# laomao0/BIN

Hardware: AMD Instinct MI355X
Metric: interpolated frames/sec at 1280x720 (higher is better)
Workload: dtype f16x3 (fp16 hi+lo pairs = 22-bit significands, 3 MFMA products, f32 accumulate; fp32-class: 1e-6 vs the fp32 reference); 1 GPU; Adobe240 test_blur 1280x720 inference, batch=1 per GPU (6-frame window padded to 768x1344 by the test.py rule), window-sharded; precision=f16x3, streams=1, pipelined_steps=False, four_call_schedule=False, parity=max-abs <= 2e-5 (f16x3) vs the fp32 reference (tests/)

## Files before the change

### bin_amd/csrc/binhip_fused_x3.hip

```cpp
#include "binhip_fused.h"
#include <type_traits>

namespace {

struct TX {
    static constexpr int R = 2, NW = 4, TH = 8, PH = 10, PW = 34;
    static constexpr int PP = (PH * PW * 2 + 63) / 64;
    static constexpr int CWP = 9, LWP = 3;
    static constexpr int PATCH_BYTES = PP * 1024;
    static constexpr int WPL = (CWP + LWP) * 1024;
    static constexpr int WBUF_BYTES = 2 * WPL;
    static constexpr int W_OFF = 2 * PATCH_BYTES;
    static constexpr int LDS_BYTES = W_OFF + 2 * WBUF_BYTES;
    static constexpr int NCHUNK = 12;
    static constexpr int NPJ = (PP + NW - 1) / NW;
    static constexpr int TAILW_OFF = W_OFF;
    static_assert(2 * LDS_BYTES <= 160 * 1024, "two workgroups per CU");
};

__device__ __forceinline__ half8 ld8(const char* p) { return *reinterpret_cast<const half8*>(p); }

__device__ __forceinline__ void tx_issue_patch(const TailKArgs& a, char* smem, int c, int pl, int wave, const unsigned* voff,
                                               long long plane_elems, unsigned plane_bytes) {
    __amdgpu_buffer_rsrc_t rs = __builtin_amdgcn_make_buffer_rsrc(
        (void*)((pl ? a.x_lo : a.x_hi) + (long long)c * plane_elems), 0, plane_bytes, 0x00020000);
    char* lds = smem + pl * TX::PATCH_BYTES;
#pragma unroll
    for (int j = 0; j < TX::NPJ; ++j) {
        const int i = wave + TX::NW * j;
        if (i < TX::PP) __builtin_amdgcn_raw_ptr_buffer_load_lds(rs, (lds_void_t*)(lds + i * 1024), 16, voff[j], 0, 0, 0);
    }
}

__device__ __forceinline__ void tx_issue_weights(const TailKArgs& a, char* smem, int c, int buf, int wave, int lane) {
    __amdgpu_buffer_rsrc_t ch = __builtin_amdgcn_make_buffer_rsrc((void*)(a.wc_hi + (long long)c * (9 * 32 * 16)), 0, 9 * 1024, 0x00020000);
    __amdgpu_buffer_rsrc_t cl = __builtin_amdgcn_make_buffer_rsrc((void*)(a.wc_lo + (long long)c * (9 * 32 * 16)), 0, 9 * 1024, 0x00020000);
    __amdgpu_buffer_rsrc_t lh = __builtin_amdgcn_make_buffer_rsrc((void*)(a.wl_hi + (long long)c * (96 * 16)), 0, 3 * 1024, 0x00020000);
    __amdgpu_buffer_rsrc_t ll = __builtin_amdgcn_make_buffer_rsrc((void*)(a.wl_lo + (long long)c * (96 * 16)), 0, 3 * 1024, 0x00020000);
    char* lds = smem + TX::W_OFF + buf * TX::WBUF_BYTES;
    const unsigned v = (unsigned)(lane * 16);
#pragma unroll
    for (int j = 0; j < 6; ++j) {
        const int i = wave + TX::NW * j;
        const int pl = i >= 12 ? 1 : 0;
        const int k = i - 12 * pl;
        const bool lff = k >= TX::CWP;
        const int t = lff ? k - TX::CWP : k;
        __builtin_amdgcn_raw_ptr_buffer_load_lds(pl ? (lff ? ll : cl) : (lff ? lh : ch), (lds_void_t*)(lds + i * 1024), 16, v,
                                                 t * 1024, 0, 0);
    }
}

__device__ __forceinline__ void tx_issue_tailw(const TailKArgs& a, char* smem, int wave, int lane) {
    __amdgpu_buffer_rsrc_t lh = __builtin_amdgcn_make_buffer_rsrc((void*)(a.wl_hi + (long long)12 * (96 * 16)), 0, 6 * 1024, 0x00020000);
    __amdgpu_buffer_rsrc_t ll = __builtin_amdgcn_make_buffer_rsrc((void*)(a.wl_lo + (long long)12 * (96 * 16)), 0, 6 * 1024, 0x00020000);
    char* lds = smem + TX::TAILW_OFF;
#pragma unroll
    for (int j = 0; j < 3; ++j) {
        const int i = wave + TX::NW * j;
        const int pl = i >= 6 ? 1 : 0;
        __builtin_amdgcn_raw_ptr_buffer_load_lds(pl ? ll : lh, (lds_void_t*)(lds + i * 1024), 16, (unsigned)(lane * 16),
                                                 (i - 6 * pl) * 1024, 0, 0);
    }
}

template <int RES>
__device__ __forceinline__ void tx_add_residual_row(const half8& bc, floatx16 (&accl)[3][TX::R], int r) {
    constexpr int K = RES >> 1, HF = RES & 1;
    union H8 { half8 h; unsigned u[4]; };
    H8 v;
    v.h = bc;
#pragma unroll
    for (int k = 0; k < 2; ++k) {
        auto sw = __builtin_amdgcn_permlane32_swap(v.u[k], v.u[2 + k], false, false);
        v.u[k] = sw[0]; v.u[2 + k] = sw[1];
    }
#pragma unroll
    for (int ge = 0; ge < 2; ++ge)
#pragma unroll
        for (int j = 0; j < 4; ++j) accl[K][r][4 * (2 * HF + ge) + j] += (float)v.h[4 * ge + j];
}

template <bool HI, int RES>
__device__ __forceinline__ void tx_compute(const char* pb, const char* wb, int a_lane_off, int b_lane_off,
                                           floatx16 (&accc)[TX::R], floatx16 (&accl)[3][TX::R], half8 (&carry)[TX::R]) {
    constexpr int R = TX::R;
    constexpr int NSTEP = 12;
    half8 B[2][R + 2];
    half8 Ah[2], Al[2];
    auto load_b = [&](int dx, half8 (&dst)[R + 2]) {
#pragma unroll
// ... 25 lines not shown
        if constexpr (RES >= 0) {
            if (s == 0) {
#pragma unroll
                for (int r = 0; r < R; ++r) tx_add_residual_row<RES>(carry[r], accl, r);
                __builtin_amdgcn_sched_barrier(0);
            }
        }
        if (!lff) {
            const int set = dx & 1;
            if constexpr (HI) {
#pragma unroll
                for (int r = 0; r < R; ++r)
                    accc[r] = __builtin_amdgcn_mfma_f32_32x32x16_f16(Al[s & 1], B[set][r + k], accc[r], 0, 0, 0);
            }
#pragma unroll
            for (int r = 0; r < R; ++r)
                accc[r] = __builtin_amdgcn_mfma_f32_32x32x16_f16(Ah[s & 1], B[set][r + k], accc[r], 0, 0, 0);
        } else {
            if constexpr (HI) {
#pragma unroll
                for (int r = 0; r < R; ++r)
                    accl[k][r] = __builtin_amdgcn_mfma_f32_32x32x16_f16(Al[s & 1], B[1][r + 1], accl[k][r], 0, 0, 0);
            }
#pragma unroll
            for (int r = 0; r < R; ++r)
                accl[k][r] = __builtin_amdgcn_mfma_f32_32x32x16_f16(Ah[s & 1], B[1][r + 1], accl[k][r], 0, 0, 0);
        }
        __builtin_amdgcn_sched_barrier(0);
    }
#pragma unroll
    for (int r = 0; r < R; ++r) carry[r] = B[1][r + 1];
}

__global__ void __launch_bounds__(256) __attribute__((amdgpu_waves_per_eu(2, 2)))
rdb_tail_x3_kernel(const TailKArgs a, const float* __restrict__ bias_c, const float* __restrict__ bias_l) {
    extern __shared__ __attribute__((aligned(16))) char smem[];
    BH_TL_DECL;
    BH_TL_BEGIN();
    const int tid = threadIdx.x;
    const int lane = tid & 63;
    const int wave = __builtin_amdgcn_readfirstlane(tid >> 6);
    const int n = lane & 31, kg = lane >> 5;

    int bid = blockIdx.x;
    if (a.xcd_remap) bid = xcd_band(bid, gridDim.x);
    const int tx = bid % a.tiles_x;
    bid /= a.tiles_x;
    const int ty = bid % a.tiles_y;
    const int img = bid / a.tiles_y;
    const int tx0 = tx * 32, ty0 = ty * TX::TH;
    const int H = a.H, W = a.W;
    const long long plane_elems = (long long)a.N * H * W * 16;
    const unsigned plane_bytes = (unsigned)(plane_elems * 2);

    unsigned voff[TX::NPJ];
#pragma unroll
    for (int j = 0; j < TX::NPJ; ++j) {
        const int i = wave + TX::NW * j;
        const int q = i * 64 + lane;
        const int cg = q >= TX::PH * TX::PW ? 1 : 0;
        const int p = q - cg * (TX::PH * TX::PW);
        const int py = p / TX::PW, px = p - py * TX::PW;
        const int gy = ty0 + py - 1, gx = tx0 + px - 1;
        const bool ok = (p < TX::PH * TX::PW) && gy >= 0 && gy < H && gx >= 0 && gx < W;
        voff[j] = ok ? (unsigned)((((long long)img * H + gy) * W + gx) * 32 + cg * 16) : 0x80000000u;
    }

    floatx16 accc[TX::R];
    floatx16 accl[3][TX::R];
#pragma unroll
    for (int r = 0; r < TX::R; ++r)
#pragma unroll
        for (int e = 0; e < 16; ++e) {
            accc[r][e] = 0.f;
            accl[0][r][e] = 0.f; accl[1][r][e] = 0.f; accl[2][r][e] = 0.f;
        }
    const int a_lane_off = n * 32 + ((kg ^ ((n >> 3) & 1)) << 4);
    const int b_lane_off = (kg * (TX::PH * TX::PW) + wave * TX::R * TX::PW + n) * 16;

    __builtin_amdgcn_s_setprio(2);
    tx_issue_weights(a, smem, 0, 0, wave, lane);
    tx_issue_patch(a, smem, 0, 0, wave, voff, plane_elems, plane_bytes);
    half8 carry[TX::R];
    auto chunk = [&](const int c, auto res_hi, auto res_lo) __attribute__((always_inline)) {
        constexpr int RH = decltype(res_hi)::value, RL = decltype(res_lo)::value;
        const char* wb = smem + TX::W_OFF + (c & 1) * TX::WBUF_BYTES;
        wait_vmcnt<0>();
        __builtin_amdgcn_s_barrier();
        __builtin_amdgcn_sched_barrier(0);
#if BINHIP_TIMELINE
        if (c == 0) BH_TL_STAMP(1);
#endif
        tx_issue_patch(a, smem, c, 1, wave, voff, plane_elems, plane_bytes);
        if (c + 1 < TX::NCHUNK) tx_issue_weights(a, smem, c + 1, (c + 1) & 1, wave, lane);
        else tx_issue_tailw(a, smem, wave, lane);
        tx_compute<true, RH>(smem, wb, a_lane_off, b_lane_off, accc, accl, carry);
        wait_vmcnt<0>();
        __builtin_amdgcn_s_barrier();
        __builtin_amdgcn_sched_barrier(0);
        if (c + 1 < TX::NCHUNK) tx_issue_patch(a, smem, c + 1, 0, wave, voff, plane_elems, plane_bytes);
        tx_compute<false, RL>(smem + TX::PATCH_BYTES, wb, a_lane_off, b_lane_off, accc, accl, carry);
    };
    using std::integral_constant;
    chunk(0, integral_constant<int, -1>{}, integral_constant<int, 0>{});
    chunk(1, integral_constant<int, 0>{}, integral_constant<int, 1>{});
    chunk(2, integral_constant<int, 1>{}, integral_constant<int, 2>{});
    chunk(3, integral_constant<int, 2>{}, integral_constant<int, 3>{});
    chunk(4, integral_constant<int, 3>{}, integral_constant<int, 4>{});
    chunk(5, integral_constant<int, 4>{}, integral_constant<int, 5>{});
    chunk(6, integral_constant<int, 5>{}, integral_constant<int, -1>{});
    for (int c = 7; c < TX::NCHUNK; ++c) chunk(c, integral_constant<int, -1>{}, integral_constant<int, -1>{});
    wait_vmcnt<0>();
    __builtin_amdgcn_s_barrier();
    __builtin_amdgcn_sched_barrier(0);

    __builtin_amdgcn_s_setprio(0);
    const int gx = tx0 + n;
    union H4 { half4 h; unsigned u[2]; };
    union H8 { half8 h; unsigned u[4]; };
    unsigned sat = 0;
    half8 Bh[2][TX::R], Bl[2][TX::R];
#pragma unroll
    for (int r = 0; r < TX::R; ++r) {
        const int gy = ty0 + wave * TX::R + r;
        const bool ok = (gy < H) && (gx < W);
#pragma unroll
        for (int gp = 0; gp < 2; ++gp) {
            H4 hv[2], lv[2];
#pragma unroll
            for (int ge = 0; ge < 2; ++ge) {
                const int g = 2 * gp + ge;
                float b8[8];
#pragma unroll
                for (int j = 0; j < 8; ++j) b8[j] = bias_c[8 * g + j];
                const float v[4] = {accc[r][4 * g + 0] + (kg ? b8[4] : b8[0]), accc[r][4 * g + 1] + (kg ? b8[5] : b8[1]),
                                    accc[r][4 * g + 2] + (kg ? b8[6] : b8[2]), accc[r][4 * g + 3] + (kg ? b8[7] : b8[3])};
                split_pair(v[0], v[1], sat, hv[ge].u[0], lv[ge].u[0], true);
                split_pair(v[2], v[3], sat, hv[ge].u[1], lv[ge].u[1], true);
            }
#pragma unroll
            for (int k = 0; k < 2; ++k) {
                auto sw = __builtin_amdgcn_permlane32_swap(hv[0].u[k], hv[1].u[k], false, false);
                hv[0].u[k] = sw[0]; hv[1].u[k] = sw[1];
                auto sl = __builtin_amdgcn_permlane32_swap(lv[0].u[k], lv[1].u[k], false, false);
                lv[0].u[k] = sl[0]; lv[1].u[k] = sl[1];
            }
            H8 fh, fl;
            fh.u[0] = hv[0].u[0]; fh.u[1] = hv[0].u[1]; fh.u[2] = hv[1].u[0]; fh.u[3] = hv[1].u[1];
            fl.u[0] = lv[0].u[0]; fl.u[1] = lv[0].u[1]; fl.u[2] = lv[1].u[0]; fl.u[3] = lv[1].u[1];
            Bh[gp][r] = fh.h;
            Bl[gp][r] = fl.h;
            if (a.o3_hi && ok) {
                const long long o = (long long)gp * plane_elems + ((((long long)img * H + gy) * W + gx) << 4) + kg * 8;
                *reinterpret_cast<uint4*>(a.o3_hi + o) = make_uint4(fh.u[0], fh.u[1], fh.u[2], fh.u[3]);
                *reinterpret_cast<uint4*>(a.o3_lo + o) = make_uint4(fl.u[0], fl.u[1], fl.u[2], fl.u[3]);
            }
        }
    }

    const char* tailw = smem + TX::TAILW_OFF;
#pragma unroll
    for (int t = 0; t < 2; ++t) {
#pragma unroll
        for (int mt = 0; mt < 3; ++mt) {
            const int off = (t * 96 + mt * 32) * 32 + a_lane_off;
            const half8 Ah = ld8(tailw + off);
            const half8 Al = ld8(tailw + 6 * 1024 + off);
#pragma unroll
            for (int r = 0; r < TX::R; ++r) {
                accl[mt][r] = __builtin_amdgcn_mfma_f32_32x32x16_f16(Al, Bh[t][r], accl[mt][r], 0, 0, 0);
                accl[mt][r] = __builtin_amdgcn_mfma_f32_32x32x16_f16(Ah, Bh[t][r], accl[mt][r], 0, 0, 0);
                accl[mt][r] = __builtin_amdgcn_mfma_f32_32x32x16_f16(Ah, Bl[t][r], accl[mt][r], 0, 0, 0);
            }
        }
    }
    if (a.flags && __builtin_amdgcn_ballot_w64(sat != 0) != 0 && lane == 0) atomicOr(a.flags, BINHIP_FLAG_SATURATED);
    BH_TL_STAMP(2);

    ConvKArgs e;
    e.bias = a.bl; e.y_hi = a.y_hi; e.y_lo = a.y_lo;
    e.r_hi = e.r_lo = e.r2_hi = e.r2_lo = e.m_hi = nullptr;
    e.flags = a.flags;
    e.N = a.N; e.H = H; e.W = W;
    e.relu = 0; e.has_res = 0; e.cout = 96; e.wt = a.wt;
    e.och_limit = 6; e.res_chunks = 0; e.mask_from = 0; e.y_cpg = 0; e.y_cpg_inv = 0; e.y_group_stride = 0; e.y_unshuf = 0;
    conv_epilogue<3, TX::R, 3, BINHIP_EPI_PLANES, false>(e, bias_l, accl, img, ty0 + wave * TX::R, tx0, 0, true, n, kg, plane_elems);
    BH_TL_FINISH(a, blockIdx.x);
}

}

int bh_launch_tail_x3(const TailKArgs& a0, hipStream_t s) {
    static std::atomic<unsigned long long> lds_set{0};
    if (int rc = bh_set_max_lds(&rdb_tail_x3_kernel, TX::LDS_BYTES, lds_set)) return rc;
    TailKArgs a = a0;
    a.tiles_x = (a.W + 31) / 32;
    a.tiles_y = (a.H + TX::TH - 1) / TX::TH;
#if BINHIP_TIMELINE
    a.tl = bh_tl_reserve((unsigned)(a.tiles_x * a.tiles_y * a.N), &a.tl_base);
    a.tl_launch = (2u << 24) | (g_bh_tl_serial.fetch_add(1) & 0xFFFFFFu);
#endif
    rdb_tail_x3_kernel<<<dim3((unsigned)(a.tiles_x * a.tiles_y * a.N)), dim3(256), TX::LDS_BYTES, s>>>(a, a.bc, a.bl);
    BH_CHECK_LAUNCH();
    return 0;
}
```

### bin_amd/csrc/binhip_conv_common.h

```cpp
#pragma once
#include "binhip_internal.h"
#ifndef BINHIP_TIMELINE
#define BINHIP_TIMELINE 0
#endif

typedef _Float16 half8 __attribute__((ext_vector_type(8)));
typedef _Float16 half4 __attribute__((ext_vector_type(4)));
typedef float floatx16 __attribute__((ext_vector_type(16)));
typedef float floatx4 __attribute__((ext_vector_type(4)));
typedef __attribute__((address_space(3))) void lds_void_t;
typedef unsigned u32x4 __attribute__((ext_vector_type(4)));

int bh_launch_upnet_ring(const void* x_hi, const void* x_lo, const float* wvar, const float* bvar, float* out, const float* const* images,
                         int nimg, int N, int H, int W, int cin, hipStream_t s);
int bh_upnet_gsub(const float* g, int N, int H, int W, const float* scale, void* y_hi, void* y_lo, void* status, hipStream_t s);
int bh_upnet_ring_dgrad(const float* g, const float* wvar, const float* scale, void* gx_hi, void* gx_lo, void* status, int N, int H, int W,
                        int cin, hipStream_t s);
int bh_upnet_ring_wgrad(const float* g, const void* x_hi, const void* x_lo, float* dwvar, float* dbvar, int N, int H, int W, int cin,
                        int accumulate, hipStream_t s);
struct ConvKArgs {
    const _Float16* x_hi;
    const _Float16* x_lo;
    const _Float16* w_hi;
    const _Float16* w_lo;
// ... 96 lines not shown
__device__ __forceinline__ void wait_vmcnt() {
    asm volatile("s_waitcnt vmcnt(%0)" ::"n"(N) : "memory");
}

__device__ __forceinline__ void store16(_Float16* base, long long off_elems, uint4 v, int wt) {
    if (wt) {
        __amdgpu_buffer_rsrc_t rs = __builtin_amdgcn_make_buffer_rsrc((void*)base, 0, 0xFFFFFFFFu, 0x00020000);
        u32x4 d = {v.x, v.y, v.z, v.w};
        __builtin_amdgcn_raw_buffer_store_b128(d, rs, (int)(off_elems * 2), 0, 16);
    } else {
        *reinterpret_cast<uint4*>(base + off_elems) = v;
    }
}

__device__ __forceinline__ int xcd_band(int bid, int nwg) {
    const int q = nwg >> 3, r = nwg & 7, xcd = bid & 7, k = bid >> 3;
    return (xcd < r ? xcd * (q + 1) : r * (q + 1) + (xcd - r) * q) + k;
}

template <int MT, int R, int NT, int EPI, bool XTRA>
__device__ __forceinline__ void conv_epilogue(const ConvKArgs& a, const float* __restrict__ bias, floatx16 (&acc)[MT][R],
                                              int img, int row0, int tx0, int co0, bool first_col, int n, int kg,
                                              long long plane_elems) {
    const int H = a.H, W = a.W;
    const int gx = tx0 + n;
    auto bias4 = [&](int co_u, float (&bv)[4]) {
        float b8[8];
#pragma unroll
        for (int j = 0; j < 8; ++j) b8[j] = bias[co_u + j];
#pragma unroll
        for (int j = 0; j < 4; ++j) bv[j] = kg ? b8[4 + j] : b8[j];
    };
    if constexpr (EPI == BINHIP_EPI_FINAL_SUBPIX) {
        const int ncolour = a.cout >> 2;
        const int H2 = 2 * H, W2 = 2 * W;
        float bv[2][4];
        bias4(co0, bv[0]);
        bias4(co0 + 8, bv[1]);
        const bool col_ok = first_col && (gx < W);
        float sum[R][2][4];
#pragma unroll
        for (int r = 0; r < R; ++r) {
            const int gy = row0 + r;
#pragma unroll
            for (int g = 0; g < 2; ++g) {
                const int c = 2 * g + kg;
                const bool ok = col_ok && gy < H && c < ncolour;
#pragma unroll
                for (int q = 0; q < 4; ++q) {
                    float sj = 0.f;
                    if (ok && a.nimg > 0) {
                        const long long idx = (((long long)img * ncolour + c) * H2 + 2 * gy + (q >> 1)) * W2 + 2 * gx + (q & 1);
                        sj = a.img[0][idx];
                        for (int t = 1; t < a.nimg; ++t) sj += a.img[t][idx];
                        sj = sj / (float)a.nimg;
                    }
                    sum[r][g][q] = sj;
                }
            }
        }
#pragma unroll
        for (int r = 0; r < R; ++r) {
            const int gy = row0 + r;
#pragma unroll
            for (int g = 0; g < 2; ++g) {
                const int c = 2 * g + kg;
                if (!(col_ok && gy < H && c < ncolour)) continue;
#pragma unroll
                for (int q = 0; q < 4; ++q) {
                    const long long idx = (((long long)img * ncolour + c) * H2 + 2 * gy + (q >> 1)) * W2 + 2 * gx + (q & 1);
                    a.out_f32[idx] = (acc[0][r][4 * g + q] + bv[g][q]) + sum[r][g][q];
                }
            }
        }
    } else if constexpr (EPI == BINHIP_EPI_FINAL) {
        float bv[4];
        bias4(co0, bv);
        const bool mine = (kg == 0) && first_col && (gx < W);
        float sum[R][4];
#pragma unroll
        for (int r = 0; r < R; ++r) {
            const int gy = row0 + r;
#pragma unroll
            for (int j = 0; j < 4; ++j) {
                float sj = 0.f;
                if (mine && gy < H && j < a.cout && a.nimg > 0) {
                    const long long idx = (((long long)img * a.cout + j) * H + gy) * W + gx;
                    sj = a.img[0][idx];
                    for (int t = 1; t < a.nimg; ++t) sj += a.img[t][idx];
                    sj = sj / (float)a.nimg;
                }
                sum[r][j] = sj;
            }
        }
#pragma unroll
        for (int r = 0; r < R; ++r) {
            const int gy = row0 + r;
            if (!(mine && gy < H)) continue;
#pragma unroll
            for (int j = 0; j < 4; ++j) {
                if (j >= a.cout) break;
                const long long idx = (((long long)img * a.cout + j) * H + gy) * W + gx;
                a.out_f32[idx] = (acc[0][r][j] + bv[j]) + sum[r][j];
            }
// ... 246 lines not shown
```

### bin_amd/csrc/binhip_conv_x3.hip

```cpp
#include "binhip_conv_common.h"
constexpr int X3_R = 2, X3_WN = 8;

template <int KS, int R, int WN>
struct X3Cfg {
    static constexpr int PAD = KS / 2;
    static constexpr int TH = R * WN;
    static constexpr int PH = TH + KS - 1;
    static constexpr int PW = 32 + KS - 1;
    static constexpr int PP = (PH * PW * 2 + 63) / 64;
    static constexpr int WP = KS * KS;
    static constexpr int NW = WN;
    static constexpr int PATCH_BYTES = PP * 1024;
    static constexpr int WBUF_BYTES = 2 * WP * 1024;
    static constexpr int LDS_BYTES = 2 * PATCH_BYTES + 2 * WBUF_BYTES;
    static constexpr int NPJ = (PP + NW - 1) / NW;
    static constexpr int NWJ = (2 * WP + NW - 1) / NW;
    static_assert((KS == 3 ? 2 : 1) * LDS_BYTES <= 160 * 1024, "LDS budget");
};

template <class C>
__device__ __forceinline__ void x3_issue_patch(const ConvKArgs& a, char* smem, int c, int pl, int buf, int wave,
                                               const unsigned* voff, long long plane_elems, unsigned plane_bytes) {
    const _Float16* xb = pl ? a.x_lo : a.x_hi;
    const long long coff = (a.cpg > 0) ? (long long)(c / a.cpg) * a.group_stride + (long long)(c % a.cpg) * plane_elems
                                       : (long long)c * plane_elems;
    __amdgpu_buffer_rsrc_t rs = __builtin_amdgcn_make_buffer_rsrc((void*)(xb + coff), 0, plane_bytes, 0x00020000);
    char* lds = smem + buf * C::PATCH_BYTES;
#pragma unroll
    for (int j = 0; j < C::NPJ; ++j) {
        const int i = wave + C::NW * j;
        if ((C::PP % C::NW == 0) || (i < C::PP))
            __builtin_amdgcn_raw_ptr_buffer_load_lds(rs, (lds_void_t*)(lds + i * 1024), 16, voff[j], 0, 0, 0);
    }
}

template <class C, int KS>
__device__ __forceinline__ void x3_issue_weights(const ConvKArgs& a, char* smem, int c, int buf, int wave, int lane, int z) {
    const long long woff = ((long long)z * a.nchunks + c) * (KS * KS * 32 * 16);
    __amdgpu_buffer_rsrc_t wh = __builtin_amdgcn_make_buffer_rsrc((void*)(a.w_hi + woff), 0, KS * KS * 1024, 0x00020000);
    __amdgpu_buffer_rsrc_t wl = __builtin_amdgcn_make_buffer_rsrc((void*)(a.w_lo + woff), 0, KS * KS * 1024, 0x00020000);
    char* lds = smem + 2 * C::PATCH_BYTES + buf * C::WBUF_BYTES;
#pragma unroll
    for (int j = 0; j < C::NWJ; ++j) {
        const int i = wave + C::NW * j;
        if (((2 * C::WP) % C::NW == 0) || (i < 2 * C::WP)) {
            const bool lo = i >= C::WP;
            const int t = lo ? i - C::WP : i;
            __builtin_amdgcn_raw_ptr_buffer_load_lds(lo ? wl : wh, (lds_void_t*)(lds + i * 1024), 16,
                                                     (unsigned)(lane * 16), t * 1024, 0, 0);
        }
    }
}

__device__ __forceinline__ half8 x3_ld8(const char* p) { return *reinterpret_cast<const half8*>(p); }
__device__ __forceinline__ floatx16 x3_mfma(half8 a, half8 b, floatx16 c) {
    return __builtin_amdgcn_mfma_f32_32x32x16_f16(a, b, c, 0, 0, 0);
}

template <class C, int KS, int R, bool HI>
__device__ __forceinline__ void x3_compute(const char* pb, const char* wb, int a_lane_off, int b_lane_off, floatx16 (&acc)[R]) {
    constexpr int NTAP = KS * KS;
    half8 B[2][R + KS - 1];
    half8 Ah[2], Al[2];
    auto load_b = [&](int dx, half8 (&dst)[R + KS - 1]) {
#pragma unroll
        for (int rr = 0; rr < R + KS - 1; ++rr) dst[rr] = x3_ld8(pb + b_lane_off + (rr * C::PW + dx) * 16);
    };
    auto load_a = [&](int s, half8& h, half8& l) {
        const int dx = s / KS, dy = s % KS;
        const int off = ((dy * KS + dx) * 32) * 32 + a_lane_off;
        h = x3_ld8(wb + off);
        if constexpr (HI) l = x3_ld8(wb + C::WP * 1024 + off);
    };
    load_b(0, B[0]);
    load_a(0, Ah[0], Al[0]);
#pragma unroll
    for (int s = 0; s < NTAP; ++s) {
        const int dx = s / KS, dy = s % KS;
        if (s + 1 < NTAP) load_a(s + 1, Ah[(s + 1) & 1], Al[(s + 1) & 1]);
        if (dy == 0 && dx + 1 < KS) load_b(dx + 1, B[(dx + 1) & 1]);
        __builtin_amdgcn_sched_barrier(0);
        if constexpr (HI) {
#pragma unroll
// ... 69 lines not shown
    const int n = lane & 31;
    const int kg = lane >> 5;
    const int tx0 = tx * 32, ty0 = ty * C::TH;
    const int H = a.H, W = a.W;
    const long long plane_elems = (long long)a.N * H * W * 16;
    const unsigned plane_bytes = (unsigned)(plane_elems * 2);

    unsigned voff[C::NPJ];
#pragma unroll
    for (int j = 0; j < C::NPJ; ++j) {
        const int i = wave + C::NW * j;
        const int q = i * 64 + lane;
        const int cg = q >= C::PH * C::PW ? 1 : 0;
        const int p = q - cg * (C::PH * C::PW);
        const int py = p / C::PW;
        const int px = p - py * C::PW;
        const int gy = ty0 + py - C::PAD;
        const int gx = tx0 + px - C::PAD;
        const bool ok = (p < C::PH * C::PW) && (gy >= 0) && (gy < H) && (gx >= 0) && (gx < W);
        voff[j] = ok ? (unsigned)((((long long)img * H + gy) * W + gx) * 32 + cg * 16) : 0x80000000u;
    }

    floatx16 acc[1][R];
#pragma unroll
    for (int r = 0; r < R; ++r)
#pragma unroll
        for (int e = 0; e < 16; ++e) acc[0][r][e] = 0.f;

    const int nchunks = a.nchunks;
    const int a_lane_off = n * 32 + ((kg ^ ((n >> 3) & 1)) << 4);
    const int b_lane_off = (kg * (C::PH * C::PW) + wave * R * C::PW + n) * 16;

    __builtin_amdgcn_s_setprio(2);
    x3_issue_weights<C, KS>(a, smem, 0, 0, wave, lane, z);
    if constexpr (GATED) {
        if (gate.chunk <= 0 && gate.flags) {
            if (tid < 9) {
                const int ny = ty + tid / 3 - 1, nx = tx + tid % 3 - 1;
                if (ny >= 0 && ny < a.tiles_y && nx >= 0 && nx < a.tiles_x) {
                    const unsigned* f = gate.flags + ((size_t)img * a.tiles_y + ny) * a.tiles_x + nx;
                    unsigned spins = 0;
                    while (__hip_atomic_load(f, __ATOMIC_RELAXED, __HIP_MEMORY_SCOPE_AGENT) != gate.epoch) {
                        __builtin_amdgcn_s_sleep(2);
                        if (++spins > RDB3_SPIN_LIMIT) {
                            if (gate.status) atomicOr(gate.status, BINHIP_STATUS_SYNC_TIMEOUT);
                            break;
                        }
                    }
                }
            }
            __builtin_amdgcn_s_barrier();
            __builtin_amdgcn_sched_barrier(0);
        }
    }
    x3_issue_patch<C>(a, smem, 0, 0, 0, wave, voff, plane_elems, plane_bytes);
    for (int c = 0; c < nchunks; ++c) {
        const char* wb = smem + 2 * C::PATCH_BYTES + (c & 1) * C::WBUF_BYTES;
        if (a.prog_prio) {
            const int q = (4 * c) / nchunks;
            if (q == 0) __builtin_amdgcn_s_setprio(3);
            else if (q == 1) __builtin_amdgcn_s_setprio(2);
            else if (q == 2) __builtin_amdgcn_s_setprio(1);
            else __builtin_amdgcn_s_setprio(0);
        }
        wait_vmcnt<0>();
        __builtin_amdgcn_s_barrier();
        __builtin_amdgcn_sched_barrier(0);
#if BINHIP_TIMELINE
        if (c == 0) BH_TL_STAMP(1);
#endif
        x3_issue_patch<C>(a, smem, c, 1, 1, wave, voff, plane_elems, plane_bytes);
        if (c + 1 < nchunks) x3_issue_weights<C, KS>(a, smem, c + 1, (c + 1) & 1, wave, lane, z);
        unsigned gate_seen = gate.epoch;
        const unsigned* gate_word = nullptr;
        if constexpr (GATED) {
            if (c + 1 == gate.chunk && gate.flags && tid < 9) {
                const int ny = ty + tid / 3 - 1, nx = tx + tid % 3 - 1;
                if (ny >= 0 && ny < a.tiles_y && nx >= 0 && nx < a.tiles_x) {
                    gate_word = gate.flags + ((size_t)img * a.tiles_y + ny) * a.tiles_x + nx;
                    gate_seen = __hip_atomic_load(gate_word, __ATOMIC_RELAXED, __HIP_MEMORY_SCOPE_AGENT);
                }
            }
        }
        const bool pair = (KS == 5) && !XTRA && a.half_last && (c + 1 == nchunks);
        if constexpr (KS == 5 && !XTRA) {
            if (pair) x3_compute_pair<C, KS, R, true>(smem, wb, n, kg, wave, acc[0]);
            else x3_compute<C, KS, R, true>(smem, wb, a_lane_off, b_lane_off, acc[0]);
        } else {
            x3_compute<C, KS, R, true>(smem, wb, a_lane_off, b_lane_off, acc[0]);
        }
        wait_vmcnt<0>();
        __builtin_amdgcn_s_barrier();
        __builtin_amdgcn_sched_barrier(0);
        if constexpr (GATED) {
            if (c + 1 == gate.chunk && gate.flags) {
                if (gate_word) {
                    unsigned spins = 0;
                    while (gate_seen != gate.epoch) {
                        __builtin_amdgcn_s_sleep(2);
                        gate_seen = __hip_atomic_load(gate_word, __ATOMIC_RELAXED, __HIP_MEMORY_SCOPE_AGENT);
                        if (++spins > RDB3_SPIN_LIMIT) {
                            if (gate.status) atomicOr(gate.status, BINHIP_STATUS_SYNC_TIMEOUT);
                            break;
                        }
                    }
                }
                __builtin_amdgcn_s_barrier();
                __builtin_amdgcn_sched_barrier(0);
            }
        }
        if (c + 1 < nchunks) x3_issue_patch<C>(a, smem, c + 1, 0, 0, wave, voff, plane_elems, plane_bytes);
        if constexpr (KS == 5 && !XTRA) {
            if (pair) x3_compute_pair<C, KS, R, false>(smem + C::PATCH_BYTES, wb, n, kg, wave, acc[0]);
            else x3_compute<C, KS, R, false>(smem + C::PATCH_BYTES, wb, a_lane_off, b_lane_off, acc[0]);
        } else {
            x3_compute<C, KS, R, false>(smem + C::PATCH_BYTES, wb, a_lane_off, b_lane_off, acc[0]);
        }
    }
    BH_TL_STAMP(2);
    __builtin_amdgcn_s_setprio(0);
    conv_epilogue<1, R, 3, EPI, XTRA>(a, bias, acc, img, ty0 + wave * R, tx0, z * 32, z == 0, n, kg, plane_elems);
    BH_TL_FINISH(a, (((img * a.tiles_y + ty) * a.tiles_x + tx) * a.ncol + z));
}

template <int KS, int R, int WN, int EPI, int WIDE, bool XTRA>
__global__ void __launch_bounds__(64 * WN)
    __attribute__((amdgpu_waves_per_eu((KS == 5 && !XTRA) ? WN / 4 : WN / 2, (KS == 5 && !XTRA) ? WN / 4 : WN / 2)))
conv_x3_kernel(const ConvKArgs a, const float* __restrict__ bias) {
    extern __shared__ __attribute__((aligned(16))) char smem[];
    int bid = blockIdx.x;
    if (a.xcd_remap) bid = xcd_band(bid, gridDim.x);
    const int ncol = a.ncol;
    const int z = bid % ncol;
    bid /= ncol;
    const int tx = bid % a.tiles_x;
    bid /= a.tiles_x;
    const int ty = bid % a.tiles_y;
    const int img = bid / a.tiles_y;
    x3_tile<KS, R, WN, EPI, XTRA>(a, bias, smem, img, ty, tx, z);
}

struct Rdb3Args {
    ConvKArgs conv[3];
    unsigned* flags;
    unsigned epoch;
    int T;
};

template <int R, int WN>
__global__ void __launch_bounds__(64 * WN) __attribute__((amdgpu_waves_per_eu(WN / 2, WN / 2)))
conv_x3_rdbs_kernel(const Rdb3Args a, const float* __restrict__ bias0, const float* __restrict__ bias1,
                    const float* __restrict__ bias2) {
    extern __shared__ __attribute__((aligned(16))) char smem[];
    const int tiles_x = a.conv[0].tiles_x, tiles_y = a.conv[0].tiles_y;
    const int G = (int)gridDim.x;
    const int b = xcd_band((int)blockIdx.x, G);
#pragma unroll 1
    for (int p = 0; p < 3; ++p) {
        const ConvKArgs& ka = a.conv[p];
        const float* bias = p == 0 ? bias0 : (p == 1 ? bias1 : bias2);
        X3Gate gate;
        gate.flags = p > 0 ? a.flags + (size_t)(p - 1) * a.T : nullptr;
        gate.epoch = a.epoch;
        gate.chunk = ka.nchunks - 2;
        gate.status = ka.flags;
#pragma unroll 1
        for (int t0 = b; t0 < a.T; t0 += G) {
            int t = t0;
            const int tx = t % tiles_x;
            t /= tiles_x;
            const int ty = t % tiles_y;
            const int img = t / tiles_y;
            x3_tile<3, R, WN, BINHIP_EPI_PLANES, false, true>(ka, bias, smem, img, ty, tx, 0, gate);
            asm volatile("s_waitcnt vmcnt(0)" ::: "memory");
            __syncthreads();
            if (threadIdx.x == 0 && p < 2)
                __hip_atomic_store(a.flags + (size_t)p * a.T + t0, a.epoch, __ATOMIC_RELAXED, __HIP_MEMORY_SCOPE_AGENT);
        }
    }
}

template <int KS, int R, int WN, int EPI, int WIDE, bool XTRA>
static int launch_x3_x(const ConvKArgs& ka, int cout_pad, hipStream_t s) {
    using C = X3Cfg<KS, R, WN>;
    static std::atomic<unsigned long long> lds_set{0};
    if (int rc = bh_set_max_lds(&conv_x3_kernel<KS, R, WN, EPI, WIDE, XTRA>, C::LDS_BYTES, lds_set)) return rc;
    ConvKArgs a = ka;
    a.tiles_x = (a.W + 31) / 32;
    a.tiles_y = (a.H + C::TH - 1) / C::TH;
    a.ncol = cout_pad / 32;
    dim3 grid((unsigned)(a.tiles_x * a.tiles_y * a.N * a.ncol));
    a.prog_prio = (KS == 3 && !XTRA && (long long)grid.x <= 2ll * binhip_device_cus()) ? 1 : 0;
#if BINHIP_TIMELINE
    a.tl = bh_tl_reserve(grid.x, &a.tl_base);
    a.tl_launch = ((KS == 3 && EPI == BINHIP_EPI_PLANES && WIDE == 0 && !XTRA ? 1u : 3u) << 24) | (g_bh_tl_serial.fetch_add(1) & 0xFFFFFFu);
#endif
    conv_x3_kernel<KS, R, WN, EPI, WIDE, XTRA><<<grid, dim3(64 * C::NW), C::LDS_BYTES, s>>>(a, a.bias);
    BH_CHECK_LAUNCH();
    return 0;
}
template <int KS, int R, int WN, int EPI, int WIDE>
static int launch_x3(const ConvKArgs& ka, int cout_pad, hipStream_t s) {
    if constexpr (EPI == BINHIP_EPI_PLANES) {
        if (ka.has_res || ka.r2_hi || ka.m_hi || ka.y_unshuf) return launch_x3_x<KS, R, WN, EPI, WIDE, true>(ka, cout_pad, s);
    }
    return launch_x3_x<KS, R, WN, EPI, WIDE, false>(ka, cout_pad, s);
}

int bh_launch_rdb3_x3(const ConvKArgs* convs, unsigned* flags, unsigned epoch, int cus, hipStream_t s) {
    using C = X3Cfg<3, X3_R, X3_WN>;
    static std::atomic<unsigned long long> lds_set{0};
    static std::atomic<int> per_cu{-1};
    if (int rc = bh_set_max_lds(&conv_x3_rdbs_kernel<X3_R, X3_WN>, C::LDS_BYTES, lds_set)) return rc;
    int occ = per_cu.load(std::memory_order_acquire);
    if (occ < 0) {
        int n = 0;
        hipError_t e = hipOccupancyMaxActiveBlocksPerMultiprocessor(&n, conv_x3_rdbs_kernel<X3_R, X3_WN>, 64 * C::NW,
                                                                    C::LDS_BYTES);
        if (e != hipSuccess) return (int)e;
        occ = n > 2 ? 2 : n;
        per_cu.store(occ, std::memory_order_release);
    }
// ... 305 lines not shown

int bh_launch_final_m16(const ConvKArgs& ka, hipStream_t s) {
    using C = X3Cfg<3, 2, 8>;
    static std::atomic<unsigned long long> lds_set{0};
    if (ka.nchunks * 9 > M16::WPIECES * 8) return BINHIP_E_SHAPE;
    if (int rc = bh_set_max_lds(&final_m16_kernel, M16::LDS_BYTES, lds_set)) return rc;
    ConvKArgs a = ka;
    a.tiles_x = (a.W + 31) / 32;
    a.tiles_y = (a.H + C::TH - 1) / C::TH;
    a.ncol = 1;
    final_m16_kernel<<<dim3((unsigned)(a.tiles_x * a.tiles_y * a.N)), dim3(512), M16::LDS_BYTES, s>>>(a, a.bias);
    BH_CHECK_LAUNCH();
    return 0;
}

int bh_launch_final_dot2(const ConvKArgs& ka, hipStream_t s) {
    using C = X3Cfg<3, 2, 4>;
    ConvKArgs a = ka;
    a.tiles_x = (a.W + 31) / 32;
    a.tiles_y = (a.H + C::TH - 1) / C::TH;
    a.ncol = 1;
    dim3 grid((unsigned)(a.tiles_x * a.tiles_y * a.N));
    const unsigned* wh = reinterpret_cast<const unsigned*>(a.w_hi);
    final_dot2_kernel<1><<<grid, dim3(256), 2 * C::PATCH_BYTES, s>>>(a, wh, wh);
    BH_CHECK_LAUNCH();
    return 0;
}

int bh_launch_conv_x3_k5(const ConvKArgs& a, int cout_pad, hipStream_t s) {
    return launch_x3<5, X3_R, X3_WN, BINHIP_EPI_PLANES, 1>(a, cout_pad, s);
}

int bh_launch_conv_x3_k5_subpix(const ConvKArgs& a, hipStream_t s) {
    return launch_x3<5, X3_R, X3_WN, BINHIP_EPI_FINAL_SUBPIX, 0>(a, 32, s);
}

struct RingArgs {
    const _Float16* x_hi;
    const _Float16* x_lo;
    const float* wvar;
    const float* bvar;
    float* out;
    const float* img[5];
    int N, H, W, cin, nimg;
};
constexpr int RING_THREADS = 128;
__global__ void __launch_bounds__(RING_THREADS) upnet_ring_kernel(const RingArgs a) {
    __shared__ float red[3][RING_THREADS / 64];
    const int tid = threadIdx.x, lane = tid & 63, wave = tid >> 6;
    const int H = a.H, W = a.W, H2 = 2 * H, W2 = 2 * W;
    const int ring = 2 * W2 + 2 * (H2 - 2);
    int id = blockIdx.x;
    const int img = id / ring;
    id -= img * ring;
    int Y, X;
    if (id < W2) { Y = 0; X = id; }
    else if (id < 2 * W2) { Y = H2 - 1; X = id - W2; }
    else { const int k = id - 2 * W2; Y = 1 + (k >> 1); X = (k & 1) ? W2 - 1 : 0; }
    const int y = Y >> 1, i = Y & 1, x = X >> 1, j = X & 1;
    const int vy = (Y == 0) ? 0 : (Y == H2 - 1 ? 2 : 1), vx = (X == 0) ? 0 : (X == W2 - 1 ? 2 : 1);
    const int var = 3 * vy + vx, sub = 2 * i + j;
    const int cin = a.cin, ng = cin >> 3, items = 25 * ng;
    const long long wstride = (long long)25 * cin;
    const float* w = a.wvar + ((long long)var * 12 + sub) * wstride;
    float s0 = 0.f, s1 = 0.f, s2 = 0.f;
    for (int it = tid; it < items; it += RING_THREADS) {
        const int tap = it / ng, ci = (it - tap * ng) << 3;
// ... 65 lines not shown
```

Measured before the change: 16.27 interpolated frames/s.

## Deepen tail kernel patch ring to three slots for two-ahead prefetch

Turns the RDB tail x3 kernel's patch double buffer into a templated ring of two or three slots. The three-slot version packs each slot to the exact plane size and trims the last load piece to fit. It prefetches two sub-stages ahead and waits on partial vmcnt counts instead of draining all loads, so global latency overlaps the MFMA work. The host checks occupancy and falls back to the two-slot kernel if three slots would drop below two workgroups per CU; the cost is more LDS and fragile per-wave vmcnt bookkeeping.

```diff
diff --git a/bin_amd/csrc/binhip_fused_x3.hip b/bin_amd/csrc/binhip_fused_x3.hip
--- a/bin_amd/csrc/binhip_fused_x3.hip
+++ b/bin_amd/csrc/binhip_fused_x3.hip
@@ -7,40 +7,57 @@
     static constexpr int R = 2, NW = 4, TH = 8, PH = 10, PW = 34;
     static constexpr int PP = (PH * PW * 2 + 63) / 64;
     static constexpr int CWP = 9, LWP = 3;
-    static constexpr int PATCH_BYTES = PP * 1024;
+    static constexpr int PLANE_BYTES = PH * PW * 32;
+    static constexpr int LAST_LANES = (PLANE_BYTES - (PP - 1) * 1024) / 16;
     static constexpr int WPL = (CWP + LWP) * 1024;
     static constexpr int WBUF_BYTES = 2 * WPL;
-    static constexpr int W_OFF = 2 * PATCH_BYTES;
-    static constexpr int LDS_BYTES = W_OFF + 2 * WBUF_BYTES;
     static constexpr int NCHUNK = 12;
     static constexpr int NPJ = (PP + NW - 1) / NW;
+    static constexpr int WJ = 6, TWJ = 3;
+    static_assert(NW * (NPJ - 1) <= PP - 1 && PP - 1 < NW * NPJ, "only a wave's last patch piece can be the short one");
+    static_assert(WJ * NW == 2 * (CWP + LWP) && TWJ * NW == 4 * LWP, "weight pieces divide evenly over the waves");
+};
+
+template <int NSLOT>
+struct TXL {
+    static_assert(NSLOT == 2 || NSLOT == 3, "patch ring of two (one sub-stage ahead) or three (two ahead) slots");
+    static constexpr bool PACKED = NSLOT == 3;
+    static constexpr int PATCH_BYTES = PACKED ? TX::PLANE_BYTES : TX::PP * 1024;
+    static constexpr int W_OFF = NSLOT * PATCH_BYTES;
+    static constexpr int LDS_BYTES = W_OFF + 2 * TX::WBUF_BYTES;
     static constexpr int TAILW_OFF = W_OFF;
+    static_assert(PATCH_BYTES % 16 == 0, "ds_read_b128 alignment of every slot");
     static_assert(2 * LDS_BYTES <= 160 * 1024, "two workgroups per CU");
 };
 
 __device__ __forceinline__ half8 ld8(const char* p) { return *reinterpret_cast<const half8*>(p); }
 
-__device__ __forceinline__ void tx_issue_patch(const TailKArgs& a, char* smem, int c, int pl, int wave, const unsigned* voff,
+template <bool PACKED>
+__device__ __forceinline__ void tx_issue_patch(const TailKArgs& a, char* lds, int c, int pl, int wave, int lane, const unsigned* voff,
                                                long long plane_elems, unsigned plane_bytes) {
     __amdgpu_buffer_rsrc_t rs = __builtin_amdgcn_make_buffer_rsrc(
         (void*)((pl ? a.x_lo : a.x_hi) + (long long)c * plane_elems), 0, plane_bytes, 0x00020000);
-    char* lds = smem + pl * TX::PATCH_BYTES;
 #pragma unroll
     for (int j = 0; j < TX::NPJ; ++j) {
         const int i = wave + TX::NW * j;
-        if (i < TX::PP) __builtin_amdgcn_raw_ptr_buffer_load_lds(rs, (lds_void_t*)(lds + i * 1024), 16, voff[j], 0, 0, 0);
-    }
-}
-
-__device__ __forceinline__ void tx_issue_weights(const TailKArgs& a, char* smem, int c, int buf, int wave, int lane) {
+        if (j < TX::NPJ - 1 || i < TX::PP - 1 || (!PACKED && i == TX::PP - 1)) {
+            __builtin_amdgcn_raw_ptr_buffer_load_lds(rs, (lds_void_t*)(lds + i * 1024), 16, voff[j], 0, 0, 0);
+        } else if (i == TX::PP - 1) {
+            if (lane < TX::LAST_LANES)
+                __builtin_amdgcn_raw_ptr_buffer_load_lds(rs, (lds_void_t*)(lds + i * 1024), 16, voff[j], 0, 0, 0);
+        }
+    }
+}
+
+__device__ __forceinline__ void tx_issue_weights(const TailKArgs& a, char* wring, int c, int buf, int wave, int lane) {
     __amdgpu_buffer_rsrc_t ch = __builtin_amdgcn_make_buffer_rsrc((void*)(a.wc_hi + (long long)c * (9 * 32 * 16)), 0, 9 * 1024, 0x00020000);
     __amdgpu_buffer_rsrc_t cl = __builtin_amdgcn_make_buffer_rsrc((void*)(a.wc_lo + (long long)c * (9 * 32 * 16)), 0, 9 * 1024, 0x00020000);
     __amdgpu_buffer_rsrc_t lh = __builtin_amdgcn_make_buffer_rsrc((void*)(a.wl_hi + (long long)c * (96 * 16)), 0, 3 * 1024, 0x00020000);
     __amdgpu_buffer_rsrc_t ll = __builtin_amdgcn_make_buffer_rsrc((void*)(a.wl_lo + (long long)c * (96 * 16)), 0, 3 * 1024, 0x00020000);
-    char* lds = smem + TX::W_OFF + buf * TX::WBUF_BYTES;
+    char* lds = wring + buf * TX::WBUF_BYTES;
     const unsigned v = (unsigned)(lane * 16);
 #pragma unroll
-    for (int j = 0; j < 6; ++j) {
+    for (int j = 0; j < TX::WJ; ++j) {
         const int i = wave + TX::NW * j;
         const int pl = i >= 12 ? 1 : 0;
         const int k = i - 12 * pl;
@@ -51,12 +68,11 @@
     }
 }
 
-__device__ __forceinline__ void tx_issue_tailw(const TailKArgs& a, char* smem, int wave, int lane) {
+__device__ __forceinline__ void tx_issue_tailw(const TailKArgs& a, char* lds, int wave, int lane) {
     __amdgpu_buffer_rsrc_t lh = __builtin_amdgcn_make_buffer_rsrc((void*)(a.wl_hi + (long long)12 * (96 * 16)), 0, 6 * 1024, 0x00020000);
     __amdgpu_buffer_rsrc_t ll = __builtin_amdgcn_make_buffer_rsrc((void*)(a.wl_lo + (long long)12 * (96 * 16)), 0, 6 * 1024, 0x00020000);
-    char* lds = smem + TX::TAILW_OFF;
-#pragma unroll
-    for (int j = 0; j < 3; ++j) {
+#pragma unroll
+    for (int j = 0; j < TX::TWJ; ++j) {
         const int i = wave + TX::NW * j;
         const int pl = i >= 6 ? 1 : 0;
         __builtin_amdgcn_raw_ptr_buffer_load_lds(pl ? ll : lh, (lds_void_t*)(lds + i * 1024), 16, (unsigned)(lane * 16),
@@ -148,8 +164,10 @@
     for (int r = 0; r < R; ++r) carry[r] = B[1][r + 1];
 }
 
+template <int NSLOT>
 __global__ void __launch_bounds__(256) __attribute__((amdgpu_waves_per_eu(2, 2)))
 rdb_tail_x3_kernel(const TailKArgs a, const float* __restrict__ bias_c, const float* __restrict__ bias_l) {
+    using L = TXL<NSLOT>;
     extern __shared__ __attribute__((aligned(16))) char smem[];
     BH_TL_DECL;
     BH_TL_BEGIN();
@@ -195,27 +213,50 @@
     const int b_lane_off = (kg * (TX::PH * TX::PW) + wave * TX::R * TX::PW + n) * 16;
 
     __builtin_amdgcn_s_setprio(2);
-    tx_issue_weights(a, smem, 0, 0, wave, lane);
-    tx_issue_patch(a, smem, 0, 0, wave, voff, plane_elems, plane_bytes);
+    char* const wring = smem + L::W_OFF;
+    int slot = 0;
+    auto slot_base = [&](int k) { return smem + k * L::PATCH_BYTES; };
+    auto issue_plane = [&](int s, int k) __attribute__((always_inline)) {
+        tx_issue_patch<L::PACKED>(a, slot_base(k), s >> 1, s & 1, wave, lane, voff, plane_elems, plane_bytes);
+    };
+    const bool three = wave < TX::PP - 2 * TX::NW;
+    tx_issue_weights(a, wring, 0, 0, wave, lane);
+#pragma unroll
+    for (int s = 0; s < NSLOT - 1; ++s) issue_plane(s, s);
     half8 carry[TX::R];
     auto chunk = [&](const int c, auto res_hi, auto res_lo) __attribute__((always_inline)) {
         constexpr int RH = decltype(res_hi)::value, RL = decltype(res_lo)::value;
-        const char* wb = smem + TX::W_OFF + (c & 1) * TX::WBUF_BYTES;
-        wait_vmcnt<0>();
+        const char* wb = wring + (c & 1) * TX::WBUF_BYTES;
+        const bool last = c + 1 == TX::NCHUNK;
+        if constexpr (NSLOT == 3) {
+            if (three) wait_vmcnt<3>(); else wait_vmcnt<2>();
+        } else {
+            wait_vmcnt<0>();
+        }
         __builtin_amdgcn_s_barrier();
         __builtin_amdgcn_sched_barrier(0);
 #if BINHIP_TIMELINE
         if (c == 0) BH_TL_STAMP(1);
 #endif
-        tx_issue_patch(a, smem, c, 1, wave, voff, plane_elems, plane_bytes);
-        if (c + 1 < TX::NCHUNK) tx_issue_weights(a, smem, c + 1, (c + 1) & 1, wave, lane);
-        else tx_issue_tailw(a, smem, wave, lane);
-        tx_compute<true, RH>(smem, wb, a_lane_off, b_lane_off, accc, accl, carry);
-        wait_vmcnt<0>();
+        int prev = slot == 0 ? NSLOT - 1 : slot - 1;
+        if (NSLOT == 2 || !last) issue_plane(2 * c + NSLOT - 1, prev);
+        if (!last) tx_issue_weights(a, wring, c + 1, (c + 1) & 1, wave, lane);
+        else tx_issue_tailw(a, smem + L::TAILW_OFF, wave, lane);
+        tx_compute<true, RH>(slot_base(slot), wb, a_lane_off, b_lane_off, accc, accl, carry);
+        prev = slot;
+        slot = slot + 1 == NSLOT ? 0 : slot + 1;
+        if constexpr (NSLOT == 3) {
+            if (last) wait_vmcnt<3>();
+            else if (three) wait_vmcnt<9>();
+            else wait_vmcnt<8>();
+        } else {
+            wait_vmcnt<0>();
+        }
         __builtin_amdgcn_s_barrier();
         __builtin_amdgcn_sched_barrier(0);
-        if (c + 1 < TX::NCHUNK) tx_issue_patch(a, smem, c + 1, 0, wave, voff, plane_elems, plane_bytes);
-        tx_compute<false, RL>(smem + TX::PATCH_BYTES, wb, a_lane_off, b_lane_off, accc, accl, carry);
+        if (!last) issue_plane(2 * c + NSLOT, prev);
+        tx_compute<false, RL>(slot_base(slot), wb, a_lane_off, b_lane_off, accc, accl, carry);
+        slot = slot + 1 == NSLOT ? 0 : slot + 1;
     };
     using std::integral_constant;
     chunk(0, integral_constant<int, -1>{}, integral_constant<int, 0>{});
@@ -274,7 +315,7 @@
         }
     }
 
-    const char* tailw = smem + TX::TAILW_OFF;
+    const char* tailw = smem + L::TAILW_OFF;
 #pragma unroll
     for (int t = 0; t < 2; ++t) {
 #pragma unroll
@@ -306,9 +347,29 @@
 
 }
 
+template <int NSLOT>
+static int launch_tail_x3(TailKArgs& a, hipStream_t s) {
+    using L = TXL<NSLOT>;
+    rdb_tail_x3_kernel<NSLOT><<<dim3((unsigned)(a.tiles_x * a.tiles_y * a.N)), dim3(256), L::LDS_BYTES, s>>>(a, a.bc, a.bl);
+    BH_CHECK_LAUNCH();
+    return 0;
+}
+
 int bh_launch_tail_x3(const TailKArgs& a0, hipStream_t s) {
-    static std::atomic<unsigned long long> lds_set{0};
-    if (int rc = bh_set_max_lds(&rdb_tail_x3_kernel, TX::LDS_BYTES, lds_set)) return rc;
+    static std::atomic<unsigned long long> lds_set3{0}, lds_set2{0};
+    static std::atomic<int> per_cu{-1};
+    if (int rc = bh_set_max_lds(&rdb_tail_x3_kernel<3>, TXL<3>::LDS_BYTES, lds_set3)) return rc;
+    int occ = per_cu.load(std::memory_order_acquire);
+    if (occ < 0) {
+        int n = 0;
+        hipError_t e = hipOccupancyMaxActiveBlocksPerMultiprocessor(&n, rdb_tail_x3_kernel<3>, 256, TXL<3>::LDS_BYTES);
+        if (e != hipSuccess) return (int)e;
+        occ = n;
+        per_cu.store(occ, std::memory_order_release);
+    }
+    if (occ < 2) {
+        if (int rc = bh_set_max_lds(&rdb_tail_x3_kernel<2>, TXL<2>::LDS_BYTES, lds_set2)) return rc;
+    }
     TailKArgs a = a0;
     a.tiles_x = (a.W + 31) / 32;
     a.tiles_y = (a.H + TX::TH - 1) / TX::TH;
@@ -316,7 +377,5 @@
     a.tl = bh_tl_reserve((unsigned)(a.tiles_x * a.tiles_y * a.N), &a.tl_base);
     a.tl_launch = (2u << 24) | (g_bh_tl_serial.fetch_add(1) & 0xFFFFFFu);
 #endif
-    rdb_tail_x3_kernel<<<dim3((unsigned)(a.tiles_x * a.tiles_y * a.N)), dim3(256), TX::LDS_BYTES, s>>>(a, a.bc, a.bl);
-    BH_CHECK_LAUNCH();
-    return 0;
-}
+    return occ >= 2 ? launch_tail_x3<3>(a, s) : launch_tail_x3<2>(a, s);
+}
```

Result: no change. 16.22 interpolated frames/s (-0.3%).

## Compute sub-pixel final conv as a 4x4 window per output quad instead of 5x5

Applied to the files above, without the earlier changes.

The final 5x5 conv followed by pixel shuffle is recomputed with a 4x4 tap window, shifting the output quad by one pixel. Each lane gathers a phase-specific subset of the 5x5 weights, so 16 taps are processed instead of 25, cutting MFMA work and weight/patch traffic. The one-pixel border ring is left unwritten here, presumably filled by the existing upnet ring kernel. Pairs of outputs are stored as swapped float2 writes.

```diff
diff --git a/bin_amd/csrc/binhip_conv_common.h b/bin_amd/csrc/binhip_conv_common.h
--- a/bin_amd/csrc/binhip_conv_common.h
+++ b/bin_amd/csrc/binhip_conv_common.h
@@ -152,12 +152,18 @@
         for (int j = 0; j < 4; ++j) bv[j] = kg ? b8[4 + j] : b8[j];
     };
     if constexpr (EPI == BINHIP_EPI_FINAL_SUBPIX) {
+        constexpr int SH = (NT == 3) ? 1 : 0;
         const int ncolour = a.cout >> 2;
         const int H2 = 2 * H, W2 = 2 * W;
+        auto pix = [&](int c, int gy, int q) {
+            const int Y = SH ? 2 * gy + 2 - (q >> 1) : 2 * gy + (q >> 1);
+            const int X = SH ? 2 * gx + 2 - (q & 1) : 2 * gx + (q & 1);
+            return (((long long)img * ncolour + c) * H2 + Y) * W2 + X;
+        };
         float bv[2][4];
         bias4(co0, bv[0]);
         bias4(co0 + 8, bv[1]);
-        const bool col_ok = first_col && (gx < W);
+        const bool col_ok = first_col && (gx < W - SH);
         float sum[R][2][4];
 #pragma unroll
         for (int r = 0; r < R; ++r) {
@@ -165,12 +171,12 @@
 #pragma unroll
             for (int g = 0; g < 2; ++g) {
                 const int c = 2 * g + kg;
-                const bool ok = col_ok && gy < H && c < ncolour;
+                const bool ok = col_ok && gy < H - SH && c < ncolour;
 #pragma unroll
                 for (int q = 0; q < 4; ++q) {
                     float sj = 0.f;
                     if (ok && a.nimg > 0) {
-                        const long long idx = (((long long)img * ncolour + c) * H2 + 2 * gy + (q >> 1)) * W2 + 2 * gx + (q & 1);
+                        const long long idx = pix(c, gy, q);
                         sj = a.img[0][idx];
                         for (int t = 1; t < a.nimg; ++t) sj += a.img[t][idx];
                         sj = sj / (float)a.nimg;
@@ -185,11 +191,20 @@
 #pragma unroll
             for (int g = 0; g < 2; ++g) {
                 const int c = 2 * g + kg;
-                if (!(col_ok && gy < H && c < ncolour)) continue;
-#pragma unroll
-                for (int q = 0; q < 4; ++q) {
-                    const long long idx = (((long long)img * ncolour + c) * H2 + 2 * gy + (q >> 1)) * W2 + 2 * gx + (q & 1);
-                    a.out_f32[idx] = (acc[0][r][4 * g + q] + bv[g][q]) + sum[r][g][q];
+                if (!(col_ok && gy < H - SH && c < ncolour)) continue;
+                float v[4];
+#pragma unroll
+                for (int q = 0; q < 4; ++q) v[q] = (acc[0][r][4 * g + q] + bv[g][q]) + sum[r][g][q];
+                if constexpr (SH) {
+                    typedef float float2u __attribute__((ext_vector_type(2), aligned(4)));
+#pragma unroll
+                    for (int i = 0; i < 2; ++i) {
+                        float2u w = {v[2 * i + 1], v[2 * i]};
+                        *reinterpret_cast<float2u*>(a.out_f32 + pix(c, gy, 2 * i + 1)) = w;
+                    }
+                } else {
+#pragma unroll
+                    for (int q = 0; q < 4; ++q) a.out_f32[pix(c, gy, q)] = v[q];
                 }
             }
         }
diff --git a/bin_amd/csrc/binhip_conv_x3.hip b/bin_amd/csrc/binhip_conv_x3.hip
--- a/bin_amd/csrc/binhip_conv_x3.hip
+++ b/bin_amd/csrc/binhip_conv_x3.hip
@@ -3,7 +3,7 @@
 
 template <int KS, int R, int WN>
 struct X3Cfg {
-    static constexpr int PAD = KS / 2;
+    static constexpr int PAD = (KS == 4) ? 1 : KS / 2;
     static constexpr int TH = R * WN;
     static constexpr int PH = TH + KS - 1;
     static constexpr int PW = 32 + KS - 1;
@@ -16,6 +16,7 @@
     static constexpr int NPJ = (PP + NW - 1) / NW;
     static constexpr int NWJ = (2 * WP + NW - 1) / NW;
     static_assert((KS == 3 ? 2 : 1) * LDS_BYTES <= 160 * 1024, "LDS budget");
+    static_assert(KS != 4 || (PP == 21 && LDS_BYTES == 106 * 1024), "the 4 x 4 window of a 16 x 32 tile");
 };
 
 template <class C>
@@ -49,6 +50,26 @@
             __builtin_amdgcn_raw_ptr_buffer_load_lds(lo ? wl : wh, (lds_void_t*)(lds + i * 1024), 16,
                                                      (unsigned)(lane * 16), t * 1024, 0, 0);
         }
+    }
+}
+
+template <class C>
+__device__ __forceinline__ void x3_issue_weights_subpix(const ConvKArgs& a, char* smem, int c, int buf, int wave, int lane, int z) {
+    static_assert(C::WP == 16 && (2 * C::WP) % C::NW == 0, "4 x 4 taps, hi and lo");
+    const long long woff = ((long long)z * a.nchunks + c) * (25 * 32 * 16);
+    __amdgpu_buffer_rsrc_t wh = __builtin_amdgcn_make_buffer_rsrc((void*)(a.w_hi + woff), 0, 25 * 1024, 0x00020000);
+    __amdgpu_buffer_rsrc_t wl = __builtin_amdgcn_make_buffer_rsrc((void*)(a.w_lo + woff), 0, 25 * 1024, 0x00020000);
+    char* lds = smem + 2 * C::PATCH_BYTES + buf * C::WBUF_BYTES;
+    const int co = lane >> 1;
+    const int sub = co < 12 ? 5 * ((co >> 1) & 1) + (co & 1) : 0;
+    const unsigned voff = (unsigned)(lane * 16 + sub * 1024);
+#pragma unroll
+    for (int j = 0; j < C::NWJ; ++j) {
+        const int i = wave + C::NW * j;
+        const bool lo = i >= C::WP;
+        const int t = lo ? i - C::WP : i;
+        __builtin_amdgcn_raw_ptr_buffer_load_lds(lo ? wl : wh, (lds_void_t*)(lds + i * 1024), 16, voff,
+                                                 (5 * (t >> 2) + (t & 3)) * 1024, 0, 0);
     }
 }
 
@@ -184,7 +205,11 @@
     const int b_lane_off = (kg * (C::PH * C::PW) + wave * R * C::PW + n) * 16;
 
     __builtin_amdgcn_s_setprio(2);
-    x3_issue_weights<C, KS>(a, smem, 0, 0, wave, lane, z);
+    auto issue_weights = [&](int c) __attribute__((always_inline)) {
+        if constexpr (KS == 4) x3_issue_weights_subpix<C>(a, smem, c, c & 1, wave, lane, z);
+        else x3_issue_weights<C, KS>(a, smem, c, c & 1, wave, lane, z);
+    };
+    issue_weights(0);
     if constexpr (GATED) {
         if (gate.chunk <= 0 && gate.flags) {
             if (tid < 9) {
@@ -222,7 +247,7 @@
         if (c == 0) BH_TL_STAMP(1);
 #endif
         x3_issue_patch<C>(a, smem, c, 1, 1, wave, voff, plane_elems, plane_bytes);
-        if (c + 1 < nchunks) x3_issue_weights<C, KS>(a, smem, c + 1, (c + 1) & 1, wave, lane, z);
+        if (c + 1 < nchunks) issue_weights(c + 1);
         unsigned gate_seen = gate.epoch;
         const unsigned* gate_word = nullptr;
         if constexpr (GATED) {
@@ -277,7 +302,7 @@
 
 template <int KS, int R, int WN, int EPI, int WIDE, bool XTRA>
 __global__ void __launch_bounds__(64 * WN)
-    __attribute__((amdgpu_waves_per_eu((KS == 5 && !XTRA) ? WN / 4 : WN / 2, (KS == 5 && !XTRA) ? WN / 4 : WN / 2)))
+    __attribute__((amdgpu_waves_per_eu((KS >= 4 && !XTRA) ? WN / 4 : WN / 2, (KS >= 4 && !XTRA) ? WN / 4 : WN / 2)))
 conv_x3_kernel(const ConvKArgs a, const float* __restrict__ bias) {
     extern __shared__ __attribute__((aligned(16))) char smem[];
     int bid = blockIdx.x;
@@ -338,8 +363,10 @@
     static std::atomic<unsigned long long> lds_set{0};
     if (int rc = bh_set_max_lds(&conv_x3_kernel<KS, R, WN, EPI, WIDE, XTRA>, C::LDS_BYTES, lds_set)) return rc;
     ConvKArgs a = ka;
-    a.tiles_x = (a.W + 31) / 32;
-    a.tiles_y = (a.H + C::TH - 1) / C::TH;
+    constexpr int EDGE = (KS == 4) ? 1 : 0;
+    if (a.H <= EDGE || a.W <= EDGE) return 0;
+    a.tiles_x = (a.W - EDGE + 31) / 32;
+    a.tiles_y = (a.H - EDGE + C::TH - 1) / C::TH;
     a.ncol = cout_pad / 32;
     dim3 grid((unsigned)(a.tiles_x * a.tiles_y * a.N * a.ncol));
     a.prog_prio = (KS == 3 && !XTRA && (long long)grid.x <= 2ll * binhip_device_cus()) ? 1 : 0;
@@ -711,7 +738,7 @@
 }
 
 int bh_launch_conv_x3_k5_subpix(const ConvKArgs& a, hipStream_t s) {
-    return launch_x3<5, X3_R, X3_WN, BINHIP_EPI_FINAL_SUBPIX, 0>(a, 32, s);
+    return launch_x3<4, X3_R, X3_WN, BINHIP_EPI_FINAL_SUBPIX, 0>(a, 32, s);
 }
 
 struct RingArgs {
```

Result: no change. 15.69 interpolated frames/s before, 15.78 interpolated frames/s after (median of 6 runs) (+0.5%).
